# icloud-ecnu/Prophet

Hardware: AMD Instinct MI355X
Metric: GiB/s device-resident N-way gradient-bucket sum (fp32/fp16), 1/2/4/8 GPUs (higher is better)
Workload: dtype f32

## Files before the change

prophet_amd/csrc/bpsr_k_cast.hip:

```cpp
#include <hip/hip_runtime.h>
#include <stdint.h>

#include <cstring>

#include "bpsr_kernels_impl.h"

namespace bpsr {

template <int DT>
struct Wide;

template <>
struct Wide<kFloat32> {
  using E = uint32_t;
  static constexpr int kVecs = 2;
  __device__ static uint32_t to_f32(E x) { return x; }
  __device__ static E from_f32(float f) { return bitcast<uint32_t>(f); }
  __device__ static E get(const vec16* x, int e) { return x[e >> 2].w[e & 3]; }
  __device__ static void put(vec16* x, int e, E v) { x[e >> 2].w[e & 3] = v; }
};

template <>
struct Wide<kFloat64> {
  using E = uint64_t;
  static constexpr int kVecs = 4;
  __device__ static uint32_t to_f32(E x) { return bitcast<uint32_t>((float)bitcast<double>(x)); }
  __device__ static E from_f32(float f) { return bitcast<uint64_t>((double)f); }
  __device__ static E get(const vec16* x, int e) {
    return ((uint64_t)x[e >> 1].w[(e & 1) * 2 + 1] << 32) | x[e >> 1].w[(e & 1) * 2];
  }
  __device__ static void put(vec16* x, int e, E v) {
    x[e >> 1].w[(e & 1) * 2] = (uint32_t)v;
    x[e >> 1].w[(e & 1) * 2 + 1] = (uint32_t)(v >> 32);
  }
};

template <>
struct Wide<kBFloat16> {
  using E = uint16_t;
  static constexpr int kVecs = 1;
  __device__ static uint32_t to_f32(E x) { return (uint32_t)x << 16; }
  __device__ static E from_f32(float f) { return (E)f32_to_bf16_rne(bitcast<uint32_t>(f)); }
  __device__ static E get(const vec16* x, int e) {
    return (E)(x[0].w[e >> 1] >> ((e & 1) * 16));
  }
  __device__ static void put(vec16* x, int e, E v) {
    if (e & 1) x[0].w[e >> 1] |= (uint32_t)v << 16;
    else x[0].w[e >> 1] = v;
  }
};

struct CastArgs {
  const unsigned char* src;
  unsigned char* dst;
  uint64_t n_elems;
  uint64_t head;
  uint64_t nunits;
  uint64_t tail_begin;
  uint64_t grid;
  int divisor;
  int aligned;
};

template <class W>
__device__ __forceinline__ uint16_t compress_elem(typename W::E x) {
  return (uint16_t)f2h_bits(W::to_f32(x));
}

template <class W>
__device__ __forceinline__ typename W::E decompress_elem(uint16_t h, bool div, float fd) {
  if (div) h = (uint16_t)f2h_bits(bitcast<uint32_t>((float)bitcast<_Float16>(h) / fd));
  return W::from_f32((float)bitcast<_Float16>(h));
}

template <class W>
__device__ __forceinline__ vec16 compress_unit(const vec16* x) {
  vec16 o;
#pragma unroll
  for (int e = 0; e < 8; e += 2)
    o.w[e >> 1] = (uint32_t)compress_elem<W>(W::get(x, e)) |
                  ((uint32_t)compress_elem<W>(W::get(x, e + 1)) << 16);
  return o;
}

template <class W>
__device__ __forceinline__ void decompress_unit(const vec16& h, bool div, float fd, vec16* o) {
#pragma unroll
  for (int e = 0; e < 8; ++e)
    W::put(o, e, decompress_elem<W>((uint16_t)(h.w[e >> 1] >> ((e & 1) * 16)), div, fd));
}

template <class W, bool COMPRESS, int U, int POL>
__device__ __forceinline__ void cast_tile_full(const unsigned char* src, unsigned char* dst,
                                               bool div, float fd, int lane) {
  constexpr int kAux = 2;
  constexpr int kStAux = POL == kPolWt ? 16 : kAux;
  constexpr int KV = W::kVecs;
  constexpr int kHBytes = kBlock * U * 16, kWBytes = kHBytes * KV;
  typedef uint32_t u4 __attribute__((ext_vector_type(4)));
  const auto rs = __builtin_amdgcn_make_buffer_rsrc(const_cast<unsigned char*>(src), 0,
                                                    COMPRESS ? kWBytes : kHBytes, 0x00020000);
  const auto rd = __builtin_amdgcn_make_buffer_rsrc(dst, 0, COMPRESS ? kHBytes : kWBytes,
                                                    0x00020000);
  if constexpr (COMPRESS && KV > 1) {
    constexpr int EPV = 8 / KV, DW = EPV / 2;
    const int l = lane & 63, wave0 = lane & ~63;
    vec16 x[U][KV];
#pragma unroll
    for (int j = 0; j < U; ++j)
#pragma unroll
      for (int v = 0; v < KV; ++v)
        x[j][v] = bitcast<vec16>(__builtin_amdgcn_raw_buffer_load_b128(
            rs, ((j * kBlock + wave0) * KV + v * 64 + l) * 16, 0, kAux));
    const int vi = l / (64 / KV);
#pragma unroll
    for (int j = 0; j < U; ++j) {
      uint32_t c[KV][DW];
#pragma unroll
      for (int v = 0; v < KV; ++v)
#pragma unroll
        for (int k = 0; k < DW; ++k)
          c[v][k] = (uint32_t)compress_elem<W>(W::get(&x[j][v], 2 * k)) |
                    ((uint32_t)compress_elem<W>(W::get(&x[j][v], 2 * k + 1)) << 16);
      vec16 o;
#pragma unroll
      for (int s = 0; s < KV; ++s) {
        const int from = ((l * KV + s) & 63) * 4;
#pragma unroll
        for (int k = 0; k < DW; ++k) {
          uint32_t r = (uint32_t)__builtin_amdgcn_ds_bpermute(from, (int)c[0][k]);
#pragma unroll
          for (int v = 1; v < KV; ++v) {
            const uint32_t t = (uint32_t)__builtin_amdgcn_ds_bpermute(from, (int)c[v][k]);
            r = vi == v ? t : r;
          }
          o.w[s * DW + k] = r;
        }
      }
      __builtin_amdgcn_raw_buffer_store_b128(bitcast<u4>(o), rd, (j * kBlock + lane) * 16, 0,
                                             kStAux);
    }
  } else if constexpr (COMPRESS) {
    vec16 x[U][KV];
#pragma unroll
    for (int j = 0; j < U; ++j)
#pragma unroll
      for (int v = 0; v < KV; ++v)
        x[j][v] = bitcast<vec16>(__builtin_amdgcn_raw_buffer_load_b128(
            rs, ((j * kBlock + lane) * KV + v) * 16, 0, kAux));
#pragma unroll
    for (int j = 0; j < U; ++j)
      __builtin_amdgcn_raw_buffer_store_b128(bitcast<u4>(compress_unit<W>(x[j])), rd,
                                             (j * kBlock + lane) * 16, 0, kStAux);
  } else {
    vec16 h[U];
#pragma unroll
    for (int j = 0; j < U; ++j)
      h[j] = bitcast<vec16>(
          __builtin_amdgcn_raw_buffer_load_b128(rs, (j * kBlock + lane) * 16, 0, kAux));
    if constexpr (KV > 1) {
      constexpr int EPV = 8 / KV;
      const int l = lane & 63, wave0 = lane & ~63;
#pragma unroll
      for (int j = 0; j < U; ++j) {
#pragma unroll
        for (int v = 0; v < KV; ++v) {
          const int g = v * 64 + l;
          const int from = (g / KV) * 4, sub = g % KV;
          uint32_t w[4];
#pragma unroll
          for (int k = 0; k < 4; ++k)
            w[k] = (uint32_t)__builtin_amdgcn_ds_bpermute(from, (int)h[j].w[k]);
          uint32_t d[EPV / 2];
#pragma unroll
          for (int k = 0; k < EPV / 2; ++k) {
            d[k] = w[k];
#pragma unroll
            for (int s = 1; s < KV; ++s) d[k] = sub == s ? w[s * (EPV / 2) + k] : d[k];
          }
          vec16 o{};
#pragma unroll
          for (int e = 0; e < EPV; ++e)
            W::put(&o, e, decompress_elem<W>((uint16_t)(d[e >> 1] >> ((e & 1) * 16)), div, fd));
          __builtin_amdgcn_raw_buffer_store_b128(
              bitcast<u4>(o), rd, ((j * kBlock + wave0) * KV + g) * 16, 0, kStAux);
        }
      }
      return;
    }
#pragma unroll
    for (int j = 0; j < U; ++j) {
      vec16 o[KV];
      decompress_unit<W>(h[j], div, fd, o);
#pragma unroll
      for (int v = 0; v < KV; ++v)
        __builtin_amdgcn_raw_buffer_store_b128(bitcast<u4>(o[v]), rd,
                                               ((j * kBlock + lane) * KV + v) * 16, 0, kStAux);
    }
  }
}

template <class W, bool COMPRESS, int U>
__device__ __forceinline__ void cast_tile_guarded(const unsigned char* src, unsigned char* dst,
                                                  uint64_t u0, uint64_t nunits, bool div,
                                                  float fd, int lane) {
  constexpr int KV = W::kVecs;
#pragma unroll
  for (int j = 0; j < U; ++j) {
    const uint64_t u = u0 + (uint64_t)j * kBlock + lane;
    if (u >= nunits) continue;
    if constexpr (COMPRESS) {
      vec16 x[KV];
#pragma unroll
      for (int v = 0; v < KV; ++v) x[v] = ld16<true>(src + (u * KV + v) * 16);
      st16<true>(dst + u * 16, compress_unit<W>(x));
    } else {
      vec16 o[KV];
      decompress_unit<W>(ld16<true>(src + u * 16), div, fd, o);
#pragma unroll
      for (int v = 0; v < KV; ++v) st16<true>(dst + (u * KV + v) * 16, o[v]);
    }
  }
}

template <class W, bool COMPRESS>
__device__ __forceinline__ void cast_elements(const CastArgs& a, bool div, float fd, uint64_t t,
                                              uint64_t stride) {
  using E = typename W::E;
  const bool al = a.aligned != 0;
  const uint64_t n_scalar = a.head + (a.n_elems - a.tail_begin);
  for (uint64_t s = t; s < n_scalar; s += stride) {
    const uint64_t e = s < a.head ? s : a.tail_begin + (s - a.head);
    if constexpr (COMPRESS)
      st_e<uint16_t>(a.dst + e * 2, compress_elem<W>(ld_e<E>(a.src + e * sizeof(E), al)), al);
    else
      st_e<E>(a.dst + e * sizeof(E), decompress_elem<W>(ld_e<uint16_t>(a.src + e * 2, al), div, fd),
              al);
  }
}

template <class W, bool COMPRESS, int U, int POL>
__global__ __launch_bounds__(kBlock) void cast_kernel(CastArgs a) {
  asm volatile("" ::"s"(a.src), "s"(a.dst), "s"(a.nunits), "s"(a.head), "s"(a.grid),
               "s"(a.divisor));
  constexpr uint64_t kTileUnits = (uint64_t)kBlock * U;
  constexpr uint64_t kSrcUnit = COMPRESS ? 16 * W::kVecs : 16;
  constexpr uint64_t kDstUnit = COMPRESS ? 16 : 16 * W::kVecs;
  constexpr uint64_t kSrcElem = COMPRESS ? sizeof(typename W::E) : 2;
  constexpr uint64_t kDstElem = COMPRESS ? 2 : sizeof(typename W::E);
  const bool div = !COMPRESS && a.divisor > 1;
  const float fd = (float)a.divisor;
  const uint64_t full = a.nunits / kTileUnits;
  const bool partial = full * kTileUnits < a.nunits;
  const uint64_t bid = blockIdx.x;
  const int elem_mode = a.nunits == 0 ? 2 : (bid == 0 ? 1 : 0);
  const uint64_t tile = partial ? (bid == 0 ? full : bid - 1) : bid;
  const unsigned char* vsrc = a.src + a.head * kSrcElem;
  unsigned char* vdst = a.dst + a.head * kDstElem;
  if (tile < full)
    cast_tile_full<W, COMPRESS, U, POL>(vsrc + tile * kTileUnits * kSrcUnit,
                                        vdst + tile * kTileUnits * kDstUnit, div, fd,
                                        threadIdx.x);
  else if (tile * kTileUnits < a.nunits)
    cast_tile_guarded<W, COMPRESS, U>(vsrc, vdst, tile * kTileUnits, a.nunits, div, fd,
                                      threadIdx.x);
  if (elem_mode == 2)
    cast_elements<W, COMPRESS>(a, div, fd, (uint64_t)blockIdx.x * kBlock + threadIdx.x,
                               a.grid * kBlock);
  else if (elem_mode == 1)
    cast_elements<W, COMPRESS>(a, div, fd, threadIdx.x, kBlock);
}

template <class W, bool COMPRESS, int U, int POL>
static hipError_t launch_cast_inst(const CastArgs& a, const Tuning& tu, hipStream_t s) {
  static KernelAttr attr;
  const hipError_t lds_ok =
      allow_lds(attr, reinterpret_cast<const void*>(&cast_kernel<W, COMPRESS, U, POL>));
  if (lds_ok != hipSuccess) return lds_ok;
  const int occ = a.grid >= tu.occ_min_tiles ? tu.copy_occ : 0;
  hipLaunchKernelGGL((cast_kernel<W, COMPRESS, U, POL>), dim3((uint32_t)a.grid), dim3(kBlock),
                     occ_lds_bytes(occ), s, a);
  return hipGetLastError();
}

template <class W, bool COMPRESS>
static hipError_t launch_cast_dir(const CastArgs& a, int u, int pol, const Tuning& tu,
                                  hipStream_t s) {
  if (pol == kPolWt) {
    switch (u) {
      case 1: return launch_cast_inst<W, COMPRESS, 1, kPolWt>(a, tu, s);
      case 2: return launch_cast_inst<W, COMPRESS, 2, kPolWt>(a, tu, s);
      default: return launch_cast_inst<W, COMPRESS, 4, kPolWt>(a, tu, s);
    }
  }
  switch (u) {
    case 1: return launch_cast_inst<W, COMPRESS, 1, kPolNt>(a, tu, s);
    case 2: return launch_cast_inst<W, COMPRESS, 2, kPolNt>(a, tu, s);
    default: return launch_cast_inst<W, COMPRESS, 4, kPolNt>(a, tu, s);
  }
}

static void cast_geom(const void* h, const void* w, size_t nelem, int es, CastArgs* a) {
  const uintptr_t ph = (uintptr_t)h, pw = (uintptr_t)w;
  a->n_elems = nelem;
  a->aligned = (ph % 2 == 0 && pw % (uintptr_t)es == 0) ? 1 : 0;
  a->head = a->nunits = a->tail_begin = 0;
  if (!a->aligned) return;
  const uint64_t hh = ((16 - (ph & 15)) & 15) / 2;
  const uint64_t hw = ((16 - (pw & 15)) & 15) / (uint64_t)es;
  if (hh % (16 / (uint64_t)es) != hw || hh >= nelem) return;
  a->nunits = (nelem - hh) / 8;
  if (a->nunits == 0) return;
  a->head = hh;
  a->tail_begin = hh + a->nunits * 8;
}

static hipError_t launch_cast(bool compress, void* dst, const void* src, size_t nelem, int dtype,
                              int divisor, const Tuning& tu, hipStream_t s) {
  const int es = elem_size(dtype);
  CastArgs a;
  std::memset(&a, 0, sizeof(a));
  a.src = static_cast<const unsigned char*>(src);
  a.dst = static_cast<unsigned char*>(dst);
  a.divisor = divisor;
  cast_geom(compress ? dst : src, compress ? src : dst, nelem, es, &a);
  auto tiles = [&a](int u) { return (a.nunits + (uint64_t)kBlock * u - 1) / ((uint64_t)kBlock * u); };
  int u = tu.copy_vpt;
  while (u > 1 && tiles(u) < kMinTiles) u >>= 1;
  uint64_t grid = tiles(u);
  if (grid == 0) {
    grid = (nelem + kBlock - 1) / kBlock;
    if (grid > 65536) grid = 65536;
  }
  if (grid > 0x7fffffffull) return hipErrorInvalidValue;
  a.grid = grid;
  Tuning tn = tu;
  tn.nt = 1;
  const int pol = cache_pol(tn, (uint64_t)nelem * (compress ? 2 : (uint64_t)es));
  switch (dtype) {
    case kFloat32:
      return compress ? launch_cast_dir<Wide<kFloat32>, true>(a, u, pol, tu, s)
                      : launch_cast_dir<Wide<kFloat32>, false>(a, u, pol, tu, s);
    case kFloat64:
      return compress ? launch_cast_dir<Wide<kFloat64>, true>(a, u, pol, tu, s)
                      : launch_cast_dir<Wide<kFloat64>, false>(a, u, pol, tu, s);
    case kBFloat16:
      return compress ? launch_cast_dir<Wide<kBFloat16>, true>(a, u, pol, tu, s)
                      : launch_cast_dir<Wide<kBFloat16>, false>(a, u, pol, tu, s);
    default: return hipErrorInvalidValue;
  }
}

hipError_t launch_compress_fp16(void* dst, const void* src, size_t nelem, int src_dtype,
                                const Tuning& tu, hipStream_t s) {
  return launch_cast(true, dst, src, nelem, src_dtype, 1, tu, s);
}

hipError_t launch_decompress_fp16(void* dst, const void* src, size_t nelem, int dst_dtype,
                                  int divisor, const Tuning& tu, hipStream_t s) {
  return launch_cast(false, dst, src, nelem, dst_dtype, divisor, tu, s);
}

}
```

prophet_amd/csrc/bpsr_kernels_impl.h:

```cpp
#pragma once

#include <hip/hip_ext.h>
#include <hip/hip_runtime.h>
#include <stdint.h>

#include "bpsr_internal.h"
#include "bpsr_ops.h"

namespace bpsr {

template <bool NT>
__device__ __forceinline__ vec16 ld16(const unsigned char* p) {
  typedef uint32_t u4 __attribute__((ext_vector_type(4)));
  if constexpr (NT) {
    return bitcast<vec16>(__builtin_nontemporal_load(reinterpret_cast<const u4*>(p)));
  } else {
    return bitcast<vec16>(*reinterpret_cast<const u4*>(p));
  }
}

template <bool NT>
__device__ __forceinline__ void st16(unsigned char* p, const vec16& v) {
  typedef uint32_t u4 __attribute__((ext_vector_type(4)));
  if constexpr (NT) {
    __builtin_nontemporal_store(bitcast<u4>(v), reinterpret_cast<u4*>(p));
  } else {
    *reinterpret_cast<u4*>(p) = bitcast<u4>(v);
  }
}

template <class E>
__device__ __forceinline__ E ld_e(const unsigned char* p, bool aligned) {
  if (aligned) return *reinterpret_cast<const E*>(p);
  E v;
  __builtin_memcpy(&v, p, sizeof(E));
  return v;
}

template <class E>
__device__ __forceinline__ void st_e(unsigned char* p, E v, bool aligned) {
  if (aligned) {
    *reinterpret_cast<E*>(p) = v;
  } else {
    __builtin_memcpy(p, &v, sizeof(E));
  }
}

constexpr int cmin(int a, int b) { return a < b ? a : b; }

using SrcPtrs = const unsigned char* const*;

template <class Op, bool NT, class XS = SrcPtrs>
__device__ __forceinline__ vec16 fold_vector_exact(const XS& srcs, int n, uint64_t off) {
  auto opaque = [](const unsigned char* p) {
    asm volatile("" : "+v"(p));
    return p;
  };
  typename Op::Acc acc = Op::init(ld16<NT>(opaque(srcs[0] + off)));
  for (int k = 1; k < n; ++k) Op::accum(acc, ld16<NT>(opaque(srcs[k] + off)));
  return Op::finish(acc);
}

template <class Op, int VPT, int NT, int NS, bool GUARD, class XS = SrcPtrs,
          class SP = const unsigned char* const*>
__device__ __forceinline__ void fold_tile_body(const SP& srcs, const XS& xsrcs, int n,
                                               unsigned char* dst, uint64_t vec_off,
                                               uint64_t v0, uint64_t nvec, int lane) {
  constexpr int NSA = NS < 0 ? -NS : NS;
  const int ns = NS > 0 ? NS : n;
  const uint64_t off0 = vec_off + (v0 + lane) * 16;
  constexpr uint64_t kStep = (uint64_t)kBlock * 16;
  constexpr int G = NSA > 0 ? cmin(NSA, 32 / VPT) : cmin(8, 32 / VPT);
  static_assert(NS >= 0 || G == NSA, "NS < 0 needs one load group");
  bool valid[VPT];
#pragma unroll
  for (int j = 0; j < VPT; ++j) valid[j] = !GUARD || (v0 + lane + (uint64_t)j * kBlock < nvec);
  typename Op::Acc acc[VPT];
  auto group = [&](int k0) __attribute__((always_inline)) {
    vec16 x[G][VPT];
#pragma unroll
    for (int g = 0; g < G; ++g) {
      if (NS > 0 || k0 + g < ns) {
        const unsigned char* base = srcs[k0 + g] + off0;
#pragma unroll
        for (int j = 0; j < VPT; ++j)
          x[g][j] = valid[j] ? ld16<(NT != 0)>(base + j * kStep) : vec16{{0, 0, 0, 0}};
      }
    }
#pragma unroll
    for (int g = 0; g < G; ++g) {
      if (NS > 0 || k0 + g < ns) {
#pragma unroll
        for (int j = 0; j < VPT; ++j) {
          if (k0 + g == 0) acc[j] = Op::init_fast(x[g][j]);
          else Op::fast(acc[j], x[g][j]);
        }
      }
    }
  };
  if constexpr (NSA > 0) {
#pragma unroll
    for (int k0 = 0; k0 < NSA; k0 += G) group(k0);
  } else {
    for (int k0 = 0; k0 < ns; k0 += G) group(k0);
  }
  bool bad = false;
#pragma unroll
  for (int j = 0; j < VPT; ++j) bad |= valid[j] && Op::has_nan(acc[j]);
#pragma unroll
  for (int j = 0; j < VPT; ++j) {
    vec16 out = Op::finish_fast(acc[j]);
    if (__builtin_expect(bad, 0)) {
      if (valid[j] && Op::has_nan(acc[j]))
        out = fold_vector_exact<Op, (NT != 0), XS>(xsrcs, ns, off0 + j * kStep);
    }
    if (valid[j]) st16<(NT != 0)>(dst + off0 + j * kStep, out);
  }
}

struct NoMid {
  __device__ __forceinline__ void operator()() const {}
};

template <class Op, int VPT, int NT, int NS, class Mid = NoMid, class XS = SrcPtrs,
          class SP = const unsigned char* const*>
__device__ __forceinline__ void fold_tile_full_buf(const SP& srcs, const XS& xsrcs, int n,
                                                   unsigned char* dst, uint64_t byte0, int lane,
                                                   const Mid& mid = Mid()) {
  constexpr int kAux = NT ? 2 : 0;
  constexpr int kStAux = NT == kPolWt ? 16 : kAux;
  constexpr int kTileBytes = kBlock * VPT * 16;
  constexpr int NSA = NS < 0 ? -NS : NS;
  constexpr int G = NSA > 0 ? cmin(NSA, 32 / VPT) : cmin(8, 32 / VPT);
  static_assert(NS >= 0 || G == NSA, "NS < 0 needs one load group");
  const int ns = NS > 0 ? NS : n;
  const int voff = lane * 16;
  typedef uint32_t u4 __attribute__((ext_vector_type(4)));
  auto rsrc = [&](const unsigned char* base) __attribute__((always_inline)) {
    return __builtin_amdgcn_make_buffer_rsrc(const_cast<unsigned char*>(base) + byte0, 0,
                                             kTileBytes, 0x00020000);
  };
  typename Op::Acc acc[VPT];
  auto group = [&](int k0) __attribute__((always_inline)) {
    vec16 x[G][VPT];
#pragma unroll
    for (int g = 0; g < G; ++g) {
      if (NS > 0 || k0 + g < ns) {
        const auto r = rsrc(srcs[k0 + g]);
#pragma unroll
        for (int j = 0; j < VPT; ++j)
          x[g][j] = bitcast<vec16>(__builtin_amdgcn_raw_buffer_load_b128(r, voff + j * kBlock * 16,
                                                                         0, kAux));
      }
    }
#pragma unroll
    for (int g = 0; g < G; ++g) {
      if (NS > 0 || k0 + g < ns) {
#pragma unroll
        for (int j = 0; j < VPT; ++j) {
          if (k0 + g == 0) acc[j] = Op::init_fast(x[g][j]);
          else Op::fast(acc[j], x[g][j]);
        }
      }
    }
  };
  if constexpr (NSA > 0) {
#pragma unroll
    for (int k0 = 0; k0 < NSA; k0 += G) group(k0);
  } else {
    for (int k0 = 0; k0 < ns; k0 += G) group(k0);
  }
  mid();
  bool bad = false;
#pragma unroll
  for (int j = 0; j < VPT; ++j) bad = bad || Op::has_nan(acc[j]);
  const auto rd = __builtin_amdgcn_make_buffer_rsrc(dst + byte0, 0, kTileBytes, 0x00020000);
#pragma unroll
  for (int j = 0; j < VPT; ++j) {
    vec16 out = Op::finish_fast(acc[j]);
    if (__builtin_expect(bad, 0)) {
      if (Op::has_nan(acc[j]))
        out = fold_vector_exact<Op, (NT != 0), XS>(xsrcs, ns, byte0 + voff + j * kBlock * 16);
    }
    __builtin_amdgcn_raw_buffer_store_b128(bitcast<u4>(out), rd, voff + j * kBlock * 16, 0, kStAux);
  }
}

template <class Op, int VPT, int NT, int NS>
__device__ __forceinline__ void fold_tile(const unsigned char* const* srcs, int n,
                                          unsigned char* dst, uint64_t vec_off, uint64_t v0,
                                          uint64_t nvec, int lane) {
  if (v0 + (uint64_t)kBlock * VPT <= nvec)
    fold_tile_full_buf<Op, VPT, NT, NS>(srcs, srcs, n, dst, vec_off + v0 * 16, lane);
  else
    fold_tile_body<Op, VPT, NT, NS, true>(srcs, srcs, n, dst, vec_off, v0, nvec, lane);
}

template <class Op, class XS = SrcPtrs>
__device__ __forceinline__ void fold_elements(const XS& srcs, int n,
                                              unsigned char* dst, const FoldGeom& g,
                                              bool aligned, uint64_t t, uint64_t stride) {
  using E = typename Op::E;
  const uint64_t n_head = g.head_elems;
  const uint64_t n_tail = g.n_elems - g.tail_begin;
  const uint64_t n_scalar = n_head + n_tail;
  for (uint64_t s = t; s < n_scalar; s += stride) {
    const uint64_t e = s < n_head ? s : g.tail_begin + (s - n_head);
    const bool tail = e >= g.tail_sem_from;
    const uint64_t off = e * sizeof(E);
    typename Op::EAcc acc{};
    for (int k0 = 0; k0 < n; k0 += 8) {
      E x[8];
#pragma unroll
      for (int q = 0; q < 8; ++q)
        if (k0 + q < n) x[q] = ld_e<E>(srcs[k0 + q] + off, aligned);
#pragma unroll
      for (int q = 0; q < 8; ++q) {
        if (k0 + q < n) {
          if (k0 + q == 0) acc = Op::init_e(x[q], tail);
          else Op::accum_e(acc, x[q], tail);
        }
      }
    }
    st_e<E>(dst + off, Op::finish_e(acc, tail), aligned);
  }
  if (g.copy_trailing) {
    const uint64_t tb = g.n_elems * sizeof(E);
    for (uint64_t b = t; b < g.trailing_bytes; b += stride) dst[tb + b] = srcs[0][tb + b];
  }
}

template <int NS>
__device__ __forceinline__ void pin_args(const FoldArgs& a) {
  if constexpr (NS == 8) {
    asm volatile("" ::"s"(a.srcs[0]), "s"(a.srcs[1]), "s"(a.srcs[2]), "s"(a.srcs[3]),
                 "s"(a.srcs[4]), "s"(a.srcs[5]), "s"(a.srcs[6]), "s"(a.srcs[7]), "s"(a.dst),
                 "s"(a.g.nvec), "s"(a.g.vec_off), "s"(a.grid));
  } else if constexpr (NS == 2) {
    asm volatile("" ::"s"(a.srcs[0]), "s"(a.srcs[1]), "s"(a.dst), "s"(a.g.nvec),
                 "s"(a.g.vec_off), "s"(a.grid));
  } else if constexpr (NS == 16) {
    asm volatile("" ::"s"(a.srcs[0]), "s"(a.srcs[1]), "s"(a.srcs[2]), "s"(a.srcs[3]),
                 "s"(a.srcs[4]), "s"(a.srcs[5]), "s"(a.srcs[6]), "s"(a.srcs[7]),
                 "s"(a.srcs[8]), "s"(a.srcs[9]), "s"(a.srcs[10]), "s"(a.srcs[11]),
                 "s"(a.srcs[12]), "s"(a.srcs[13]), "s"(a.srcs[14]), "s"(a.srcs[15]),
                 "s"(a.dst), "s"(a.g.nvec), "s"(a.g.vec_off), "s"(a.grid));
  } else {
    asm volatile("" ::"s"(a.dst), "s"(a.g.nvec), "s"(a.g.vec_off), "s"(a.grid));
  }
}

template <class Op, int VPT, int NT, int NS>
__global__ __launch_bounds__(kBlock) void fold_kernel(FoldArgs a) {
  pin_args<NS>(a);
  const uint64_t tile_vecs = (uint64_t)kBlock * VPT;
  const uint64_t full = a.g.nvec / tile_vecs;
  const bool partial = full * tile_vecs < a.g.nvec;
  const uint64_t bid = blockIdx.x;
  const int elem_mode = a.g.nvec == 0 ? 2 : (bid == 0 ? 1 : 0);
  const uint64_t tile = partial ? (bid == 0 ? full : bid - 1) : bid;
  if (tile < full)
    fold_tile_full_buf<Op, VPT, NT, NS>(a.srcs, a.srcs, a.n, a.dst,
                                        a.g.vec_off + tile * tile_vecs * 16, threadIdx.x);
  else if (tile * tile_vecs < a.g.nvec)
    fold_tile_body<Op, VPT, NT, NS, true>(a.srcs, a.srcs, a.n, a.dst, a.g.vec_off,
                                          tile * tile_vecs, a.g.nvec, threadIdx.x);
  if (elem_mode == 2)
    fold_elements<Op>(a.srcs, a.n, a.dst, a.g, a.aligned != 0,
                      (uint64_t)blockIdx.x * kBlock + threadIdx.x, (uint64_t)a.grid * kBlock);
  else if (elem_mode == 1)
    fold_elements<Op>(a.srcs, a.n, a.dst, a.g, a.aligned != 0, threadIdx.x, kBlock);
}

struct RecRegs {
  unsigned char* dst;
  uint32_t kind, n, a, b, c;
  const unsigned char* p[8];
};

template <class Op, int VPT, int NT, class Mid = NoMid>
__device__ __forceinline__ void run_record(const RecRegs& r, const unsigned char* const* msrcs,
                                           const BatchEntry* entries, const Mid& mid = Mid()) {
  if (r.kind == kTileElem) {
    const BatchEntry& e = entries[r.b];
    fold_elements<Op>(e.srcs, e.n, e.dst, e.g, e.aligned != 0,
                      (uint64_t)r.a * kBlock + threadIdx.x, (uint64_t)r.c * kBlock);
    mid();
  } else if (r.n <= 8) {
    if (r.kind == kTileFull) {
      fold_tile_full_buf<Op, VPT, NT, -8>(r.p, msrcs, (int)r.n, r.dst, 0, threadIdx.x, mid);
    } else {
      fold_tile_body<Op, VPT, NT, -8, true>(r.p, msrcs, (int)r.n, r.dst, 0, 0, r.a, threadIdx.x);
      mid();
    }
  } else {
    if (r.kind == kTileFull) {
      fold_tile_full_buf<Op, VPT, NT, 0>(msrcs, msrcs, (int)r.n, r.dst, 0, threadIdx.x, mid);
    } else {
      fold_tile_body<Op, VPT, NT, 0, true>(msrcs, msrcs, (int)r.n, r.dst, 0, 0, r.a,
                                           threadIdx.x);
      mid();
    }
  }
}

__device__ __forceinline__ RecRegs load_record(const unsigned char* rec) {
  const TileHead& h = *reinterpret_cast<const TileHead*>(rec);
  const unsigned char* const* msrcs =
      reinterpret_cast<const unsigned char* const*>(rec + kTileHeadBytes);
  RecRegs r;
  r.dst = h.dst;
  r.kind = h.kind;
  r.n = h.n;
  r.a = h.a;
  r.b = h.b;
  r.c = h.c;
#pragma unroll
  for (int k = 0; k < 8; ++k) r.p[k] = msrcs[k];
  asm volatile("" ::"s"(r.dst), "s"(r.kind), "s"(r.n), "s"(r.a), "s"(r.p[0]), "s"(r.p[1]),
               "s"(r.p[2]), "s"(r.p[3]), "s"(r.p[4]), "s"(r.p[5]), "s"(r.p[6]), "s"(r.p[7]));
  return r;
}

constexpr int kRecWords = (kTileHeadBytes + 8 * 8) / 4;
__device__ __forceinline__ RecRegs regs_from_words(const uint32_t* w) {
  uint32_t v[kRecWords];
#pragma unroll
  for (int k = 0; k < kRecWords; ++k) v[k] = __builtin_amdgcn_readfirstlane(w[k]);
  auto ptr = [&](int k) {
    return reinterpret_cast<unsigned char*>(((uint64_t)v[k + 1] << 32) | v[k]);
  };
  RecRegs r;
  r.dst = ptr(0);
  r.kind = v[2];
  r.n = v[3];
  r.a = v[4];
  r.b = v[5];
  r.c = v[6];
#pragma unroll
  for (int k = 0; k < 8; ++k) r.p[k] = ptr(8 + 2 * k);
  return r;
}

__device__ __forceinline__ uint32_t prefetch_record(const BatchLaunch& L, uint64_t b) {
  uint32_t v = 0;
  const uint64_t t = b + L.pf_ahead;
  if (L.pf_ahead != 0 && threadIdx.x < 2 && t < L.tiles) {
    const uint32_t* p = reinterpret_cast<const uint32_t*>(L.recs + t * L.rec_stride);
    v = p[threadIdx.x == 0 ? 0 : L.rec_stride / 4 - 1];
  }
  return v;
}
__device__ __forceinline__ void keep_prefetch(uint32_t v) { asm volatile("" ::"v"(v)); }

template <class Op, int VPT, int NT>
__global__ __launch_bounds__(kBlock) void batched_kernel(BatchLaunch L) {
  const unsigned char* rec = L.recs + (uint64_t)blockIdx.x * L.rec_stride;
  const RecRegs r = load_record(rec);
  const uint32_t pf = prefetch_record(L, blockIdx.x);
  run_record<Op, VPT, NT>(r, reinterpret_cast<const unsigned char* const*>(rec + kTileHeadBytes),
                          L.entries);
  keep_prefetch(pf);
}

__device__ __forceinline__ uint32_t ld_sys(const uint32_t* p) {
  return __hip_atomic_load(p, __ATOMIC_RELAXED, __HIP_MEMORY_SCOPE_SYSTEM);
}

__device__ __forceinline__ void note_started(const BlockqLaunch& Q) {
  if (Q.started == nullptr || threadIdx.x != 0 || blockIdx.x + kSeqLast < gridDim.x) return;
  (void)__hip_atomic_fetch_add(Q.started, 1ull, __ATOMIC_RELAXED, __HIP_MEMORY_SCOPE_SYSTEM);
}

template <class Op, int VPT, int NT>
__global__ __launch_bounds__(kBlock) void blockq_kernel(BlockqLaunch Q) {
  note_started(Q);
  __shared__ __attribute__((aligned(16))) uint32_t s_rec[2][kRecWords];
  __shared__ uint32_t s_ready, s_ready_tiles, s_abort;
  const uint32_t tid = threadIdx.x;
  const uint32_t tw = tid % (uint32_t)kRecWords;
  auto rec_at = [&](uint32_t t) { return Q.L.recs + (uint64_t)t * Q.L.rec_stride; };
  if (blockIdx.x < Q.L.tiles)
    s_rec[0][tw] = reinterpret_cast<const uint32_t*>(rec_at(blockIdx.x))[tw];
  __syncthreads();
  uint32_t ready = 0, ready_tiles = 0;
  uint32_t it = 0;
  for (uint32_t t = blockIdx.x; t < Q.L.tiles; t += Q.grid, ++it) {
    if (t >= ready_tiles) {
      if (tid < 64) {
        const uint32_t lane = tid;
        uint32_t r = ready, rt = ready_tiles;
        bool abort = false;
        const uint64_t t0 = wall_clock64();
        for (;;) {
          const uint32_t b = r + lane;
          const bool rel = b >= Q.nblocks || epoch_reached(ld_sys(Q.flags + b), Q.epoch);
          const uint64_t pending = __ballot(!rel);
          const uint32_t r2 = pending == 0 ? (r + 64 < Q.nblocks ? r + 64 : Q.nblocks)
                                           : r + (uint32_t)__builtin_ctzll(pending);
          if (r2 != r) {
            r = r2;
            rt = Q.block_first[r];
          }
          if (rt > t) break;
          if (pending == 0) continue;
          if (__hip_atomic_load(&Q.ctl->err, __ATOMIC_RELAXED, __HIP_MEMORY_SCOPE_AGENT)) {
            abort = true;
            break;
          }
          if (wall_clock64() - t0 > Q.timeout_ticks) {
            if (lane == 0)
              __hip_atomic_store(&Q.ctl->err, 1u, __ATOMIC_RELAXED, __HIP_MEMORY_SCOPE_AGENT);
            abort = true;
            break;
          }
          __builtin_amdgcn_s_sleep(4);
        }
        if (lane == 0) {
          s_ready = r;
          s_ready_tiles = rt;
          s_abort = abort ? 1u : 0u;
        }
      }
      __syncthreads();
      if (s_abort) break;
      ready = __builtin_amdgcn_readfirstlane(s_ready);
      ready_tiles = __builtin_amdgcn_readfirstlane(s_ready_tiles);
      __builtin_amdgcn_fence(__ATOMIC_ACQUIRE, "");
    }
    const uint32_t tn = t + Q.grid;
    const uint32_t w = reinterpret_cast<const uint32_t*>(rec_at(tn < Q.L.tiles ? tn : t))[tw];
    const uint32_t nslot = (it + 1) & 1;
    auto mid = [&]() __attribute__((always_inline)) { s_rec[nslot][tw] = w; };
    run_record<Op, VPT, NT>(regs_from_words(s_rec[it & 1]),
                            reinterpret_cast<const unsigned char* const*>(rec_at(t) +
                                                                          kTileHeadBytes),
                            Q.L.entries, mid);
    __syncthreads();
  }
}

__device__ __forceinline__ void forward_host_releases(const BlockqLaunch& Q) {
  if (threadIdx.x >= 64) return;
  const uint32_t lane = threadIdx.x;
  const uint64_t t0 = wall_clock64();
  for (;;) {
    bool pending = false;
    for (uint32_t base = 0; base < Q.nblocks; base += 64) {
      const uint32_t b = base + lane;
      if (b < Q.nblocks) {
        uint32_t d = ld_sys(Q.flags + b);
        const uint32_t h = ld_sys(Q.hflags + b);
        if (h != 0 && !epoch_reached(d, h)) {
          __hip_atomic_fetch_max(Q.flags + b, h, __ATOMIC_RELEASE, __HIP_MEMORY_SCOPE_SYSTEM);
          d = h;
        }
        pending = pending || !epoch_reached(d, Q.epoch);
      }
    }
    if (__ballot(pending) == 0) return;
    if (__hip_atomic_load(&Q.ctl->err, __ATOMIC_RELAXED, __HIP_MEMORY_SCOPE_AGENT)) return;
    if (wall_clock64() - t0 > Q.timeout_ticks) {
      if (lane == 0) __hip_atomic_store(&Q.ctl->err, 1u, __ATOMIC_RELAXED, __HIP_MEMORY_SCOPE_AGENT);
      return;
    }
    __builtin_amdgcn_s_sleep(2);
  }
}

template <class Op, int VPT, int NT>
__global__ __launch_bounds__(kBlock) void blockq_gate_kernel(BlockqLaunch Q) {
  note_started(Q);
  if (Q.helper && blockIdx.x == 0) {
    forward_host_releases(Q);
    return;
  }
  const uint32_t t = blockIdx.x - Q.helper;
  const uint32_t lane = threadIdx.x & 63u;
  const unsigned char* rec = Q.L.recs + (uint64_t)t * Q.L.rec_stride;
  uint32_t w = lane < Q.nblocks ? ld_sys(Q.flags + lane) : Q.epoch;
  const RecRegs r = load_record(rec);
  const uint32_t blk = reinterpret_cast<const TileHead*>(rec)->block;
  const uint32_t pf = prefetch_record(Q.L, t);
  auto released = [&](uint32_t w0) __attribute__((always_inline)) {
    if (__ballot(lane <= blk && !epoch_reached(w0, Q.epoch)) != 0) return false;
    for (uint32_t base = 64; base <= blk; base += 64) {
      const uint32_t b = base + lane;
      const uint32_t wb = b <= blk ? ld_sys(Q.flags + b) : Q.epoch;
      if (__ballot(!epoch_reached(wb, Q.epoch)) != 0) return false;
    }
    return true;
  };
  if (!released(w)) {
    const uint64_t t0 = wall_clock64();
    for (;;) {
      __builtin_amdgcn_s_sleep(4);
      w = lane < Q.nblocks ? ld_sys(Q.flags + lane) : Q.epoch;
      if (released(w)) break;
      if (__hip_atomic_load(&Q.ctl->err, __ATOMIC_RELAXED, __HIP_MEMORY_SCOPE_AGENT)) return;
      if (wall_clock64() - t0 > Q.timeout_ticks) {
        __hip_atomic_store(&Q.ctl->err, 1u, __ATOMIC_RELAXED, __HIP_MEMORY_SCOPE_AGENT);
        return;
      }
    }
    __builtin_amdgcn_fence(__ATOMIC_ACQUIRE, "");
  }
  run_record<Op, VPT, NT>(r, reinterpret_cast<const unsigned char* const*>(rec + kTileHeadBytes),
                          Q.L.entries);
  keep_prefetch(pf);
}

__device__ __forceinline__ uint64_t ld_sys64(const uint64_t* p) {
  return __hip_atomic_load(p, __ATOMIC_RELAXED, __HIP_MEMORY_SCOPE_SYSTEM);
}
__device__ __forceinline__ uint64_t ld_agent64(const uint64_t* p) {
  return __hip_atomic_load(p, __ATOMIC_RELAXED, __HIP_MEMORY_SCOPE_AGENT);
}
__device__ __forceinline__ uint32_t ld_err(const BlockqLaunch& Q) {
  return __hip_atomic_load(&Q.ctl->err, __ATOMIC_RELAXED, __HIP_MEMORY_SCOPE_AGENT);
}

__device__ __forceinline__ void forward_host_keys(const BlockqLaunch& Q) {
  const uint32_t lane = threadIdx.x & 63u;
  const uint32_t first = threadIdx.x & ~63u;
  if (first >= Q.nblocks) return;
  const uint32_t par = Q.epoch & 1u;
  const uint64_t t0 = wall_clock64();
  for (;;) {
    bool pending = false;
    const uint32_t err = ld_err(Q);
    for (uint32_t base = first; base < Q.nblocks; base += kBlock) {
      const uint32_t b = base + lane;
      if (b >= Q.nblocks) continue;
      const uint64_t d = ld_agent64(Q.kwords + (uint64_t)b * kKeyWordStride);
      const uint64_t h = ld_sys64(Q.khwords + 2 * (uint64_t)b + par);
      const uint64_t h2 =
          Q.wide ? ld_sys64(Q.khwords + 2 * (uint64_t)(Q.nblocks + b) + par) : 0;
      if ((uint32_t)d != Q.epoch) {
        if ((uint32_t)h == Q.epoch && (!Q.wide || (uint32_t)h2 == Q.epoch)) {
          if (Q.wide)
            __hip_atomic_store(Q.kwords + (uint64_t)(Q.nblocks + b) * kKeyWordStride, h2,
                               __ATOMIC_RELAXED, __HIP_MEMORY_SCOPE_AGENT);
          __hip_atomic_store(Q.kwords + (uint64_t)b * kKeyWordStride, h, __ATOMIC_RELAXED,
                             __HIP_MEMORY_SCOPE_AGENT);
#ifdef BPSR_KEYED_TRACE
          Q.ktrace[4 * (uint64_t)Q.L.tiles + b] = wall_clock64();
#endif
        } else {
          pending = true;
        }
      }
    }
    if (__ballot(pending) == 0) return;
    const bool late = wall_clock64() - t0 > Q.timeout_ticks;
    if (late || err) {
      if (lane == 0) {
        __hip_atomic_store(&Q.ctl->err, 1u, __ATOMIC_RELAXED, __HIP_MEMORY_SCOPE_AGENT);
        __hip_atomic_store(Q.herr, 1u, __ATOMIC_RELAXED, __HIP_MEMORY_SCOPE_SYSTEM);
      }
      return;
    }
    __builtin_amdgcn_s_sleep(2);
  }
}

struct PermSrcs {
  const unsigned char* const* m;
  uint32_t perm;
  __device__ __forceinline__ const unsigned char* operator[](int k) const {
    return m[(perm >> (4 * k)) & 7u];
  }
};

struct PermSrcs16 {
  const unsigned char* const* m;
  uint64_t perm;
  __device__ __forceinline__ const unsigned char* operator[](int k) const {
    return m[(perm >> (4 * k)) & 15u];
  }
};

template <int NT>
__device__ __forceinline__ void key_tile_done(const BlockqLaunch& Q, uint32_t blk,
                                              bool written_through) {
  asm volatile("s_waitcnt vmcnt(0)" ::: "memory");
  __syncthreads();
  if (threadIdx.x == 0) {
    if (!written_through) {
      __builtin_amdgcn_fence(__ATOMIC_RELEASE, "agent");
      asm volatile("s_waitcnt vmcnt(0)" ::: "memory");
    }
    const uint32_t nt = Q.block_first[blk + 1] - Q.block_first[blk];
    const uint32_t old = __hip_atomic_fetch_add(Q.kcnt + (uint64_t)blk * kKeyCntStride, 1u,
                                                __ATOMIC_RELAXED, __HIP_MEMORY_SCOPE_AGENT);
    if ((old + 1) % nt == 0)
      __hip_atomic_store(Q.khdone + blk, Q.epoch, __ATOMIC_RELAXED, __HIP_MEMORY_SCOPE_SYSTEM);
  }
}

template <class Op, int VPT, int NT>
__global__ __launch_bounds__(kBlock) void blockq_key_kernel(BlockqLaunch Q) {
  note_started(Q);
  if (Q.helper && blockIdx.x == 0) {
    forward_host_keys(Q);
    return;
  }
  const uint32_t t = blockIdx.x - Q.helper;
#ifdef BPSR_KEYED_TRACE
  unsigned long long* kt = Q.ktrace + 4 * (uint64_t)t;
  if (threadIdx.x == 0) kt[0] = wall_clock64();
#endif
  const unsigned char* rec = Q.L.recs + (uint64_t)t * Q.L.rec_stride;
  const RecRegs r = load_record(rec);
  const uint32_t blk = reinterpret_cast<const TileHead*>(rec)->block;
  const uint32_t pf = prefetch_record(Q.L, t);
  const uint64_t* wp = Q.kwords + (uint64_t)blk * kKeyWordStride;
  uint64_t w = ld_agent64(wp);
  if ((uint32_t)w != Q.epoch) {
    const uint64_t t0 = wall_clock64();
    for (;;) {
      __builtin_amdgcn_s_sleep(8);
      w = ld_agent64(wp);
      if ((uint32_t)w == Q.epoch) break;
      if (ld_err(Q)) return;
      if (wall_clock64() - t0 > Q.timeout_ticks) {
        __hip_atomic_store(&Q.ctl->err, 1u, __ATOMIC_RELAXED, __HIP_MEMORY_SCOPE_AGENT);
        return;
      }
    }
    __builtin_amdgcn_fence(__ATOMIC_ACQUIRE, "agent");
  }
#ifdef BPSR_KEYED_TRACE
  if (threadIdx.x == 0) kt[1] = wall_clock64();
#endif
  const uint32_t perm = (uint32_t)(w >> 32);
  if (perm == kKeySkip) {
    keep_prefetch(pf);
    key_tile_done<NT>(Q, blk, true);
    return;
  }
  if (Q.wide) {
    const uint64_t* hp = Q.kwords + (uint64_t)(Q.nblocks + blk) * kKeyWordStride;
    uint64_t hi = ld_agent64(hp);
    const uint64_t t0 = wall_clock64();
    while ((uint32_t)hi != Q.epoch) {
      __builtin_amdgcn_s_sleep(2);
      hi = ld_agent64(hp);
      if (wall_clock64() - t0 > Q.timeout_ticks) {
        __hip_atomic_store(&Q.ctl->err, 1u, __ATOMIC_RELAXED, __HIP_MEMORY_SCOPE_AGENT);
        return;
      }
    }
    const uint64_t perm64 = ((hi >> 32) << 32) | perm;
    const unsigned char* const* m =
        reinterpret_cast<const unsigned char* const*>(rec + kTileHeadBytes);
    const PermSrcs16 ps{m, perm64};
    if (r.kind == kTileElem) {
      const BatchEntry& e = Q.L.entries[r.b];
      fold_elements<Op, PermSrcs16>(PermSrcs16{e.srcs, perm64}, e.n, e.dst, e.g,
                                    e.aligned != 0, (uint64_t)r.a * kBlock + threadIdx.x,
                                    (uint64_t)r.c * kBlock);
    } else if (r.kind == kTileFull) {
      fold_tile_full_buf<Op, VPT, NT, 0, NoMid, PermSrcs16>(ps, ps, (int)r.n, r.dst, 0,
                                                            threadIdx.x);
    } else {
      fold_tile_body<Op, VPT, NT, 0, true, PermSrcs16>(ps, ps, (int)r.n, r.dst, 0, 0, r.a,
                                                        threadIdx.x);
    }
    keep_prefetch(pf);
    key_tile_done<NT>(Q, blk, r.kind == kTileFull && NT == kPolWt);
    return;
  }
  const unsigned char* q[8];
#pragma unroll
  for (int m = 0; m < 8; ++m) {
    const uint32_t wk = (perm >> (4 * m)) & 7u;
    const unsigned char* v = r.p[0];
#pragma unroll
    for (int k = 1; k < 8; ++k) v = wk == (uint32_t)k ? r.p[k] : v;
    q[m] = v;
  }
  const PermSrcs xs{reinterpret_cast<const unsigned char* const*>(rec + kTileHeadBytes), perm};
  if (r.kind == kTileElem) {
    const BatchEntry& e = Q.L.entries[r.b];
    fold_elements<Op, PermSrcs>(PermSrcs{e.srcs, perm}, e.n, e.dst, e.g, e.aligned != 0,
                                (uint64_t)r.a * kBlock + threadIdx.x, (uint64_t)r.c * kBlock);
  } else if (r.kind == kTileFull) {
    fold_tile_full_buf<Op, VPT, NT, -8, NoMid, PermSrcs>(q, xs, (int)r.n, r.dst, 0,
                                                         threadIdx.x);
  } else {
    fold_tile_body<Op, VPT, NT, -8, true, PermSrcs>(q, xs, (int)r.n, r.dst, 0, 0, r.a,
                                                     threadIdx.x);
  }
  keep_prefetch(pf);
#ifdef BPSR_KEYED_TRACE
  if (threadIdx.x == 0) kt[2] = wall_clock64();
#endif
  key_tile_done<NT>(Q, blk, r.kind == kTileFull && NT == kPolWt);
#ifdef BPSR_KEYED_TRACE
  if (threadIdx.x == 0) kt[3] = wall_clock64();
#endif
}


template <class K, class A>
static hipError_t launch_with_stop(K kernel, uint32_t grid, size_t lds, hipStream_t s,
                                   hipEvent_t stop, const A& arg) {
  if (stop)
    hipExtLaunchKernelGGL(kernel, dim3(grid), dim3(kBlock), (uint32_t)lds, s, nullptr, stop, 0, arg);
  else
    hipLaunchKernelGGL(kernel, dim3(grid), dim3(kBlock), lds, s, arg);
  return hipGetLastError();
}

template <class Op, int VPT, int NT, int NS>
static hipError_t launch_fold_ns(const FoldArgs& a, const Tuning& tu, hipStream_t s) {
  static KernelAttr attr;
  const hipError_t lds_ok =
      allow_lds(attr, reinterpret_cast<const void*>(&fold_kernel<Op, VPT, NT, NS>));
  if (lds_ok != hipSuccess) return lds_ok;
  FoldArgs b = a;
  b.grid = (uint32_t)fold_grid(a.g, tu, VPT);
  hipLaunchKernelGGL((fold_kernel<Op, VPT, NT, NS>), dim3(b.grid), dim3(kBlock),
                     occ_lds_bytes(launch_occ(tu, b.grid, false)), s, b);
  return hipGetLastError();
}

template <class Op, int VPT, int NT>
static hipError_t launch_fold_vpt(const FoldArgs& a, const Tuning& tu, hipStream_t s) {
  switch (a.n) {
    case 2: return launch_fold_ns<Op, VPT, NT, 2>(a, tu, s);
    case 8: return launch_fold_ns<Op, VPT, NT, 8>(a, tu, s);
    case 16: return launch_fold_ns<Op, VPT, NT, 16>(a, tu, s);
    default: return launch_fold_ns<Op, VPT, NT, 0>(a, tu, s);
  }
}

template <class Op, int NT>
static hipError_t launch_fold_pol(const FoldArgs& a, int vpt, const Tuning& tu, hipStream_t s) {
  switch (vpt) {
    case 1: return launch_fold_vpt<Op, 1, NT>(a, tu, s);
    case 4: return launch_fold_vpt<Op, 4, NT>(a, tu, s);
    default: return launch_fold_vpt<Op, 2, NT>(a, tu, s);
  }
}

template <class Op>
static hipError_t launch_fold_op(const FoldArgs& a, const Tuning& tu, hipStream_t s) {
  int vpt = fold_vpt(a.g.nvec, tu.vpt);
  const int pol = cache_pol(tu, a.g.nvec * 16);
  Tuning t = tu;
  if (pol == kPolWt && vpt == 2 && tu.occ == 1 && a.g.nvec * 16 >= kHalfTileMinBytes) {
    vpt = 1;
    t.occ = 2;
  }
  switch (pol) {
    case kPolNt: return launch_fold_pol<Op, kPolNt>(a, vpt, t, s);
    case kPolWt: return launch_fold_pol<Op, kPolWt>(a, vpt, t, s);
    default: return launch_fold_pol<Op, kPolPlain>(a, vpt, t, s);
  }
}

template <class Op, int VPT>
static hipError_t launch_batched_vpt(const BatchLaunch& L, const Tuning& tu, hipStream_t s) {
  static KernelAttr attr[3];
  const void* k[3] = {reinterpret_cast<const void*>(&batched_kernel<Op, VPT, kPolPlain>),
                      reinterpret_cast<const void*>(&batched_kernel<Op, VPT, kPolNt>),
                      reinterpret_cast<const void*>(&batched_kernel<Op, VPT, kPolWt>)};
  note_where("batched: allow_lds");
  for (int i = 0; i < 3; ++i) {
    const hipError_t ok = allow_lds(attr[i], k[i]);
    if (ok != hipSuccess) return ok;
  }
  note_where("batched: launch");
  if (L.tiles == 0) return hipSuccess;
  const size_t lds = occ_lds_bytes(launch_occ(tu, L.tiles, true));
  switch (cache_pol(tu, (uint64_t)L.tiles * VPT * kBlock * 16)) {
    case kPolNt: return launch_with_stop(batched_kernel<Op, VPT, kPolNt>, L.tiles, lds, s, L.stop, L);
    case kPolWt: return launch_with_stop(batched_kernel<Op, VPT, kPolWt>, L.tiles, lds, s, L.stop, L);
    default: return launch_with_stop(batched_kernel<Op, VPT, kPolPlain>, L.tiles, lds, s, L.stop, L);
  }
}

template <class Op>
static hipError_t launch_batched_op(const BatchLaunch& L, int vpt, const Tuning& tu,
                                    hipStream_t s) {
  switch (vpt) {
    case 1: return launch_batched_vpt<Op, 1>(L, tu, s);
    case 4: return launch_batched_vpt<Op, 4>(L, tu, s);
    default: return launch_batched_vpt<Op, 2>(L, tu, s);
  }
}

template <class Op, int VPT, int NT>
static hipError_t launch_blockq_k(const BlockqLaunch& Q, size_t lds, bool gated, hipStream_t s) {
  if (Q.keyed) {
    static KernelAttr attr_k;
    const hipError_t okk =
        allow_lds(attr_k, reinterpret_cast<const void*>(&blockq_key_kernel<Op, VPT, NT>));
    if (okk != hipSuccess) return okk;
    return launch_with_stop(blockq_key_kernel<Op, VPT, NT>, Q.grid, lds, s, Q.L.stop, Q);
  }
  if (gated) {
    static KernelAttr attr_g;
    const hipError_t okg =
        allow_lds(attr_g, reinterpret_cast<const void*>(&blockq_gate_kernel<Op, VPT, NT>));
    if (okg != hipSuccess) return okg;
    return launch_with_stop(blockq_gate_kernel<Op, VPT, NT>, Q.grid, lds, s, Q.L.stop, Q);
  }
  static KernelAttr attr_p;
  const hipError_t ok = allow_lds(attr_p, reinterpret_cast<const void*>(&blockq_kernel<Op, VPT, NT>),
                                  (int)kLdsPerCU - 256);
  if (ok != hipSuccess) return ok;
  return launch_with_stop(blockq_kernel<Op, VPT, NT>, Q.grid, lds, s, Q.L.stop, Q);
}

template <class Op, int VPT>
static hipError_t launch_blockq_vpt(const BlockqLaunch& Q, int pol, size_t lds, bool gated,
                                    hipStream_t s) {
  switch (pol) {
    case kPolNt: return launch_blockq_k<Op, VPT, kPolNt>(Q, lds, gated, s);
    case kPolWt: return launch_blockq_k<Op, VPT, kPolWt>(Q, lds, gated, s);
    default: return launch_blockq_k<Op, VPT, kPolPlain>(Q, lds, gated, s);
  }
}

template <class Op>
static hipError_t launch_blockq_op(const BlockqLaunch& Q, int vpt, int pol, size_t lds,
                                   bool gated, hipStream_t s) {
  if (Q.grid == 0) return hipSuccess;
  switch (vpt) {
    case 1: return launch_blockq_vpt<Op, 1>(Q, pol, lds, gated, s);
    case 4: return launch_blockq_vpt<Op, 4>(Q, pol, lds, gated, s);
    default: return launch_blockq_vpt<Op, 2>(Q, pol, lds, gated, s);
  }
}

}

#define BPSR_DEFINE_LAUNCHERS(NAME, OP)                                                   \
  namespace bpsr {                                                                        \
  hipError_t launch_fold_##NAME(const FoldArgs& a, const Tuning& tu, hipStream_t s) {     \
    return launch_fold_op<OP>(a, tu, s);                                                  \
  }                                                                                       \
  hipError_t launch_batched_##NAME(const BatchLaunch& L, int vpt, const Tuning& tu,      \
                                   hipStream_t s) {                                       \
    return launch_batched_op<OP>(L, vpt, tu, s);                                          \
  }                                                                                       \
  hipError_t launch_blockq_##NAME(const BlockqLaunch& Q, int vpt, int pol, size_t lds,    \
                                  bool gated, hipStream_t s) {                            \
    return launch_blockq_op<OP>(Q, vpt, pol, lds, gated, s);                               \
  }                                                                                       \
  }
```

Baseline: 5505.

## Clamp partial-tile loads via buffer rsrc, batch guarded cast loads, cap waves per EU

Adds a partial-tile fold path that builds buffer resources sized to the remaining bytes. Out-of-range lanes get their index clamped and their loads issued unconditionally, and wavefronts with no live work skip those loads entirely. The guarded cast tile now issues all loads before the compute and stores instead of interleaving per unit. The fold kernel also gets an amdgpu_waves_per_eu hint computed from the register footprint. These changes only touch tail tiles and compiler occupancy hints, so the main full-tile path is unchanged apart from register allocation.

Result: no change. 5502 (-0.0%).

```diff
diff --git a/prophet_amd/csrc/bpsr_k_cast.hip b/prophet_amd/csrc/bpsr_k_cast.hip
--- a/prophet_amd/csrc/bpsr_k_cast.hip
+++ b/prophet_amd/csrc/bpsr_k_cast.hip
@@ -205,20 +205,37 @@
                                                   uint64_t u0, uint64_t nunits, bool div,
                                                   float fd, int lane) {
   constexpr int KV = W::kVecs;
+  bool valid[U];
+  uint64_t u[U];
 #pragma unroll
   for (int j = 0; j < U; ++j) {
-    const uint64_t u = u0 + (uint64_t)j * kBlock + lane;
-    if (u >= nunits) continue;
-    if constexpr (COMPRESS) {
-      vec16 x[KV];
-#pragma unroll
-      for (int v = 0; v < KV; ++v) x[v] = ld16<true>(src + (u * KV + v) * 16);
-      st16<true>(dst + u * 16, compress_unit<W>(x));
-    } else {
+    const uint64_t idx = u0 + (uint64_t)j * kBlock + lane;
+    valid[j] = idx < nunits;
+    u[j] = valid[j] ? idx : nunits - 1;
+  }
+  if constexpr (COMPRESS) {
+    vec16 x[U][KV];
+#pragma unroll
+    for (int j = 0; j < U; ++j)
+#pragma unroll
+      for (int v = 0; v < KV; ++v) x[j][v] = ld16<true>(src + (u[j] * KV + v) * 16);
+#pragma unroll
+    for (int j = 0; j < U; ++j) {
+      const vec16 o = compress_unit<W>(x[j]);
+      if (valid[j]) st16<true>(dst + u[j] * 16, o);
+    }
+  } else {
+    vec16 h[U];
+#pragma unroll
+    for (int j = 0; j < U; ++j) h[j] = ld16<true>(src + u[j] * 16);
+#pragma unroll
+    for (int j = 0; j < U; ++j) {
       vec16 o[KV];
-      decompress_unit<W>(ld16<true>(src + u * 16), div, fd, o);
-#pragma unroll
-      for (int v = 0; v < KV; ++v) st16<true>(dst + (u * KV + v) * 16, o[v]);
+      decompress_unit<W>(h[j], div, fd, o);
+      if (valid[j]) {
+#pragma unroll
+        for (int v = 0; v < KV; ++v) st16<true>(dst + (u[j] * KV + v) * 16, o[v]);
+      }
     }
   }
 }
diff --git a/prophet_amd/csrc/bpsr_kernels_impl.h b/prophet_amd/csrc/bpsr_kernels_impl.h
--- a/prophet_amd/csrc/bpsr_kernels_impl.h
+++ b/prophet_amd/csrc/bpsr_kernels_impl.h
@@ -115,6 +115,81 @@
         out = fold_vector_exact<Op, (NT != 0), XS>(xsrcs, ns, off0 + j * kStep);
     }
     if (valid[j]) st16<(NT != 0)>(dst + off0 + j * kStep, out);
+  }
+}
+
+template <class Op, int VPT, int NT, int NS, bool GUARD, class XS = SrcPtrs,
+          class SP = const unsigned char* const*>
+__device__ __forceinline__ void fold_tile_clamped(const SP& srcs, const XS& xsrcs, int n,
+                                                  unsigned char* dst, uint64_t vec_off,
+                                                  uint64_t v0, uint64_t nvec, int lane) {
+  static_assert(GUARD, "the full tile is fold_tile_full_buf");
+  constexpr int kAux = NT ? 2 : 0;
+  constexpr int NSA = NS < 0 ? -NS : NS;
+  const int ns = NS > 0 ? NS : n;
+  constexpr int G = NSA > 0 ? cmin(NSA, 32 / VPT) : cmin(8, 32 / VPT);
+  static_assert(NS >= 0 || G == NSA, "NS < 0 needs one load group");
+  typedef uint32_t u4 __attribute__((ext_vector_type(4)));
+  const uint64_t byte0 = vec_off + v0 * 16;
+  const uint32_t left = (uint32_t)(nvec - v0);
+  auto rsrc = [&](const unsigned char* base) __attribute__((always_inline)) {
+    return __builtin_amdgcn_make_buffer_rsrc(const_cast<unsigned char*>(base) + byte0, 0,
+                                             (int)(left * 16), 0x00020000);
+  };
+  bool valid[VPT];
+  int voff[VPT];
+#pragma unroll
+  for (int j = 0; j < VPT; ++j) {
+    const uint32_t idx = (uint32_t)lane + (uint32_t)j * kBlock;
+    valid[j] = idx < left;
+    voff[j] = (int)((valid[j] ? idx : left - 1) * 16);
+  }
+  const uint32_t wave0 = __builtin_amdgcn_readfirstlane((uint32_t)lane & ~63u);
+  const uint32_t live = wave0 < left ? (left - wave0 + kBlock - 1) / kBlock : 0u;
+  typename Op::Acc acc[VPT] = {};
+  auto group = [&](int k0) __attribute__((always_inline)) {
+    vec16 x[G][VPT];
+#pragma unroll
+    for (int g = 0; g < G; ++g) {
+      if (NS > 0 || k0 + g < ns) {
+        const auto r = rsrc(srcs[k0 + g]);
+#pragma unroll
+        for (int j = 0; j < VPT; ++j)
+          if ((uint32_t)j < live)
+            x[g][j] = bitcast<vec16>(__builtin_amdgcn_raw_buffer_load_b128(r, voff[j], 0, kAux));
+      }
+    }
+#pragma unroll
+    for (int g = 0; g < G; ++g) {
+      if (NS > 0 || k0 + g < ns) {
+#pragma unroll
+        for (int j = 0; j < VPT; ++j) {
+          if ((uint32_t)j < live) {
+            if (k0 + g == 0) acc[j] = Op::init_fast(x[g][j]);
+            else Op::fast(acc[j], x[g][j]);
+          }
+        }
+      }
+    }
+  };
+  if constexpr (NSA > 0) {
+#pragma unroll
+    for (int k0 = 0; k0 < NSA; k0 += G) group(k0);
+  } else {
+    for (int k0 = 0; k0 < ns; k0 += G) group(k0);
+  }
+  bool bad = false;
+#pragma unroll
+  for (int j = 0; j < VPT; ++j) bad |= valid[j] && Op::has_nan(acc[j]);
+  const auto rd = __builtin_amdgcn_make_buffer_rsrc(dst + byte0, 0, (int)(left * 16), 0x00020000);
+#pragma unroll
+  for (int j = 0; j < VPT; ++j) {
+    vec16 out = Op::finish_fast(acc[j]);
+    if (__builtin_expect(bad, 0)) {
+      if (valid[j] && Op::has_nan(acc[j]))
+        out = fold_vector_exact<Op, (NT != 0), XS>(xsrcs, ns, byte0 + (uint64_t)voff[j]);
+    }
+    if (valid[j]) __builtin_amdgcn_raw_buffer_store_b128(bitcast<u4>(out), rd, voff[j], 0, kAux);
   }
 }
 
@@ -192,8 +267,8 @@
                                           uint64_t nvec, int lane) {
   if (v0 + (uint64_t)kBlock * VPT <= nvec)
     fold_tile_full_buf<Op, VPT, NT, NS>(srcs, srcs, n, dst, vec_off + v0 * 16, lane);
-  else
-    fold_tile_body<Op, VPT, NT, NS, true>(srcs, srcs, n, dst, vec_off, v0, nvec, lane);
+  else if (v0 < nvec)
+    fold_tile_clamped<Op, VPT, NT, NS, true>(srcs, srcs, n, dst, vec_off, v0, nvec, lane);
 }
 
 template <class Op, class XS = SrcPtrs>
@@ -250,8 +325,16 @@
   }
 }
 
+constexpr int tile_waves(int VPT, int NS) {
+  const int nsa = NS < 0 ? -NS : NS;
+  const int g = nsa > 0 ? cmin(nsa, 32 / VPT) : cmin(8, 32 / VPT);
+  const int w = 512 / (g * VPT * 4 + 24);
+  return w > 8 ? 8 : (w < 1 ? 1 : w);
+}
+
 template <class Op, int VPT, int NT, int NS>
-__global__ __launch_bounds__(kBlock) void fold_kernel(FoldArgs a) {
+__global__ __launch_bounds__(kBlock) __attribute__((amdgpu_waves_per_eu(1, tile_waves(VPT, NS))))
+void fold_kernel(FoldArgs a) {
   pin_args<NS>(a);
   const uint64_t tile_vecs = (uint64_t)kBlock * VPT;
   const uint64_t full = a.g.nvec / tile_vecs;
@@ -263,8 +346,8 @@
     fold_tile_full_buf<Op, VPT, NT, NS>(a.srcs, a.srcs, a.n, a.dst,
                                         a.g.vec_off + tile * tile_vecs * 16, threadIdx.x);
   else if (tile * tile_vecs < a.g.nvec)
-    fold_tile_body<Op, VPT, NT, NS, true>(a.srcs, a.srcs, a.n, a.dst, a.g.vec_off,
-                                          tile * tile_vecs, a.g.nvec, threadIdx.x);
+    fold_tile_clamped<Op, VPT, NT, NS, true>(a.srcs, a.srcs, a.n, a.dst, a.g.vec_off,
+                                             tile * tile_vecs, a.g.nvec, threadIdx.x);
   if (elem_mode == 2)
     fold_elements<Op>(a.srcs, a.n, a.dst, a.g, a.aligned != 0,
                       (uint64_t)blockIdx.x * kBlock + threadIdx.x, (uint64_t)a.grid * kBlock);
```
